# NAIVEddd/MafrixRaytracing

Hardware: AMD Instinct MI355X
Metric: Mrays/s (primary+secondary) at 1080p/64spp; 1/2/4/8-GPU scaling (higher is better)
Workload: dtype f64; 1 GPU; C2 spot (5856 tris) + floor/light stage, 1920x1080, 64 spp per step over 1 GPU(s); scene=scenes/spot.xml, width=1920, height=1080, max_depth=3, frames_in_flight=1, pipeline=wavefront, api=mfx_trace_accumulate of the step's spp (inputs resident in HBM), parallelism=one GPU

## Files before the change

### mafrixraytracing_amd/csrc/mfx_api.cpp

```cpp
#include <dlfcn.h>

#include <mutex>
#include <set>
#include <thread>

#include "mfx_ctx.h"

using namespace mfxh;

namespace {
thread_local std::string g_err;

uint16_t half_dir(float x, bool up) {
    if (std::isinf(x)) return x > 0 ? 0x7c00 : 0xfc00;
    if (x < 0) return (uint16_t)(0x8000 | half_dir(-x, !up));
    if (x == 0) return up ? 0 : 0;
    if (x > 65504.f) return up ? 0x7c00 : 0x7bff;
    int e = 0;
    (void)std::frexp((double)x, &e);
    const int ex = std::max(e - 1, -14);
    const double ulp = std::ldexp(1.0, ex - 10);
    const double m = (double)x / ulp;
    const double k = up ? std::ceil(m) : std::floor(m);
    const double v = k * ulp;
// ... 115 lines not shown
        CK(upload(c->d_nodes_h, nh));
    }
    CK(upload(c->d_slot_ref, c->host.slot_ref));
    CK(upload(c->d_ref_blob, c->host.ref_blob));
    CK(upload(c->d_shade, c->host.shade));
    CK(upload(c->d_albedo, c->host.albedo));
    CK(upload(c->d_light, std::vector<MfxLight>{c->host.light}));
    CK(upload(c->d_cam, std::vector<MfxCamera>{c->host.camera}));
    CK(upload(c->d_refs, std::vector<const void*>{c->d_slot_ref.get(), c->d_ref_blob.get()}));
    const bool inst = !c->host.inst.empty();
    const int ninst = (int)c->host.inst.size();
    if (inst) CK(upload(c->d_inst, c->host.inst));
    const size_t npix = (size_t)c->npix, plane = sizeof(double) * npix;
    CK(c->d_accum_own.alloc(3 * npix));
    c->d_accum = c->d_accum_own;
    CK(c->d_film.alloc(3 * npix));
    CK(c->d_frame.alloc(4 * npix));
    CK(c->d_rgba.alloc(4 * npix));
    CK(c->d_work.alloc(8));
    CK(c->d_counters.alloc(WF_NCTR * WF_SHARDS));
    CK(c->d_counters_total.alloc(WF_NCTR * WF_SHARDS));
    CK(hipMemset(c->d_counters_total, 0, kCounterBytes));
    CK(c->pool.ctl.alloc(WF_CTL_ALLOC));
    size_t mfree = 0, mtotal = 0;
    if (hipMemGetInfo(&mfree, &mtotal) == hipSuccess && mfree > 0)
        c->pool.max = std::max<int64_t>(1 << 20, std::min<int64_t>(c->pool.max, (int64_t)(mfree / 4 / pool_slot_bytes(c))));
    c->pool.fail_once = getenv("MFX_POOL_FAIL_ONCE") && atoi(getenv("MFX_POOL_FAIL_ONCE")) != 0;
    if (const char* pm = getenv("MFX_POOL")) c->pool.max = std::max<int64_t>(2048, std::min<int64_t>(1 << 28, atoll(pm)));
    c->diag_iter = getenv("MFX_DIAG_ITER") != nullptr;
    c->adp.check = getenv("MFX_ADAPTIVE_CHECK") && atoi(getenv("MFX_ADAPTIVE_CHECK")) != 0;
    if (const char* e = getenv("MFX_ITER_EVENTS")) c->iter_events = atoi(e) != 0 || c->diag_iter;
    if (const char* qf = getenv("MFX_QUEUE_FROM")) c->pool.queue_from = MFX_RAY_QUEUE ? std::max(-2, atoi(qf)) : -1;
    if (const char* qc = getenv("MFX_QCHUNK")) c->pool.qchunk = std::max(64, std::min(WF_CHUNK_MAX, atoi(qc) / 64 * 64));
    if (getenv("MFX_RAY_QUEUE") && atoi(getenv("MFX_RAY_QUEUE")) == 0) c->pool.queue_from = -1;
    if (const char* ck = getenv("MFX_MEGA_CHUNK")) c->mega_chunk = std::max(1, atoi(ck));
    if (c->flags & MFX_F_IN_FLIGHT) {
        c->wf_chunk = 512;
        c->wf_shd_half = false;
    }
    if (const char* e = getenv("MFX_SHD_HALF")) c->wf_shd_half = atoi(e) != 0;
    if (const char* ck = getenv("MFX_CHUNK")) c->wf_chunk = std::max(64, std::min(WF_CHUNK_MAX, atoi(ck) / 64 * 64));
    CK(hipMemset(c->d_accum, 0, 3 * plane));
    CK(hipMemset(c->d_film, 0, 3 * plane));
    CK(hipMemset(c->d_counters, 0, kCounterBytes));
    hipDeviceProp_t prop;
    CK(hipGetDeviceProperties(&prop, c->device));
// ... 381 lines not shown
```

### mafrixraytracing_amd/csrc/mfx_ctx.h

```cpp
#pragma once
#include <hip/hip_runtime.h>
#include <rccl/rccl.h>

#include <algorithm>
#include <cmath>
#include <cstdio>
#include <cstdlib>
#include <cstring>
#include <functional>
#include <memory>
#include <string>
#include <utility>
#include <variant>
#include <vector>

#include "../../include/mafrix_rt.h"
#include "mfx_device.h"
#include "mfx_denoise.h"
#include "mfx_scene.h"
#include "mfx_wavefront.h"

namespace mfxh __attribute__((visibility("hidden"))) {

int fail(int code, const std::string& msg);
// ... 116 lines not shown
    decltype(&ncclReduce) reduce = nullptr;
    decltype(&ncclGroupStart) groupStart = nullptr;
    decltype(&ncclGroupEnd) groupEnd = nullptr;
    decltype(&ncclGetErrorString) errorString = nullptr;
};
const Rccl* rccl();

struct WfPool {
    WfParams params{};
    DevBuf<char> mem;
    int32_t slots = 0;
    size_t bytes = 0;
    bool queues = false;
    WfQueue wq[2]{};
    int queue_from = MFX_RAY_QUEUE ? -2 : -1;
    int queue_auto = 1;
    bool auto_read = false;
    bool auto_pending = false;
    int32_t qchunk = 128;
    int64_t max = 1 << 28;
    int64_t cap = 0;
    bool fail_once = false;
    DevBuf<unsigned long long> ctl;
    int queue_start() const { return queue_from == -2 ? queue_auto : queue_from; }
};

struct Ahead {
    int k = 0;
    AheadBuf ab[2];
    int nbuf = 0;
    int cap = 0;
    int cur = -1;
    int64_t last_k = -1;
    uint64_t film_epoch = 1;
    bool film_in_dfilm = true;
    int dfilm_buf = -1;
    int64_t dfilm_n = 0;
    DevBuf<unsigned long long> counters_aux;
    Event aux_ev0, aux_ev1;
    bool ready() const { return nbuf != 0; }
    void release() {
        for (AheadBuf& B : ab) B = AheadBuf{};
        counters_aux.reset(), aux_ev0.reset(), aux_ev1.reset();
        nbuf = cap = 0;
        cur = -1;
    }
// ... 169 lines not shown
```

### mafrixraytracing_amd/csrc/mfx_trace.cpp

```cpp
#include "mfx_ctx.h"

using namespace mfxh;

static int wf_ensure_pool(mfx_ctx* c, int32_t pool, bool queues) {
    WfPool& wp = c->pool;
    if (pool <= wp.slots && (!queues || wp.queues)) return MFX_OK;
    const size_t P = (size_t)pool;
    const int nv = c->host.max_depth + 1;
    const size_t per_slot = pool_slot_bytes(c) - (queues ? 0 : WF_QUEUE_BYTES_PER_SLOT);
    const size_t bytes = P * per_slot + 64 * 256;
    size_t mfree = 0, mtotal = 0, headroom = 0;
    if (hipMemGetInfo(&mfree, &mtotal) == hipSuccess && mfree > 0) {
        const size_t avail = mfree + (wp.mem ? wp.bytes : 0);
        headroom = std::min<size_t>((size_t)2 << 30, avail / 4);
        if (bytes + headroom > avail)
            return fail(MFX_E_NOMEM, "wavefront pool: " + std::to_string(bytes >> 20) + " MiB with " +
                                         std::to_string(avail >> 20) + " MiB free");
    }
    wp.mem.reset();
    wp.slots = 0;
    wp.bytes = 0;
    const hipError_t e = wp.mem.alloc(wp.fail_once ? ((size_t)1 << 50) : bytes);
    wp.fail_once = false;
    if (e != hipSuccess) {
// ... 159 lines not shown
    const int64_t ngen = (total + gen_max - 1) / gen_max;
    const int per_gen = P.max_depth + 1;
    const int iters = (int)ngen * per_gen;
    while (iter_events && (int)c->it_ev.size() < 3 * iters) {
        Event e;
        HIPCHECK(e.create());
        c->it_ev.push_back(std::move(e));
    }
    auto diag = [&](int64_t g, const char* what, int d, float fe, float fs) -> int {
        HIPCHECK(hipStreamSynchronize(c->stream));
        unsigned long long h[WF_NCTR * WF_SHARDS];
        HIPCHECK(hipMemcpy(h, c->d_counters, sizeof(h), hipMemcpyDeviceToHost));
        double r[WF_NCTR] = {0};
        for (int k = 0; k < WF_SHARDS; ++k)
            for (int q = 0; q < WF_NCTR; ++q) r[q] += (double)h[WF_NCTR * k + q];
        for (int q = WF_CTR_ITER + 1; q < WF_CTR_ITER + WF_ITER_CTRS; ++q) r[1] += r[q];
        fprintf(stderr, "gen %lld %s %d: cumulative primary %.0f ext %.0f shadow %.0f; extend %.3f ms shadow %.3f ms;"
                " stamps %.4g %.4g %.4g %.4g outer %.4g node %.4g; cumulative traversal closest %.0f %.0f %.0f"
                " shadow %.0f %.0f %.0f; scan %.4g shade %.4g lat %.4g\n", (long long)g, what, d,
                r[0], r[1], r[2], fe, fs, r[10], r[11], r[12], r[13], r[14], r[15], r[4], r[5], r[6], r[7], r[8], r[9],
                r[16], r[17], r[3]);
        return MFX_OK;
    };
    HIPCHECK(hipEventRecord(fm ? fm->e0 : c->ev0.get(), c->stream));
    int it = 0;
    for (int64_t g = 0; g < ngen; ++g) {
        P.path_base = g * gen_max;
        P.base_smp = P.path_base / per_sample;
        P.base_q = P.path_base % per_sample;
        P.total = std::min<int64_t>(gen_max, total - P.path_base);
        P.pool = (int32_t)((P.total + 4095) / 4096 * 4096);
        HIPCHECK(hipMemsetAsync(P.state, 0, sizeof(int32_t) * (size_t)P.pool, c->stream));
        for (int d = 0; d < per_gen; ++d, ++it) {
            P.start = d == 0 ? 1 : 0;
            P.iter = d;
            wf_queue_views(c, P, d);
            P.chunk = P.qcount ? wp.qchunk : chunk0;
            P.chunk_shd = (c->wf_shd_half && !P.qcount && total <= ((int64_t)1 << 25)) ? std::max(64, P.chunk / 2) : P.chunk;
            if (!iter_events) {
                HIPCHECK(mfx_wf_iteration(P, c->wf_ext_grid, c->wf_shd_grid, stats, c->stream, nullptr));
                continue;
            }
            const Event* ev = c->it_ev.data() + 3 * it;
            hipEvent_t mid = ev[1];
            HIPCHECK(hipEventRecord(ev[0], c->stream));
            HIPCHECK(mfx_wf_iteration(P, c->wf_ext_grid, c->wf_shd_grid, stats, c->stream, &mid));
            HIPCHECK(hipEventRecord(ev[2], c->stream));
            if (c->diag_iter) {
                HIPCHECK(hipStreamSynchronize(c->stream));
                float fe = 0.f, fs = 0.f;
                HIPCHECK(hipEventElapsedTime(&fe, ev[0], ev[1]));
                HIPCHECK(hipEventElapsedTime(&fs, ev[1], ev[2]));
                MFX_TRY(diag(g, "iter", d + 1, fe, fs));
            }
        }
        wf_queue_views(c, P, -1);
        if (split && g == ngen - 1) {
            const int tiles_x = (W + 7) / 8;
            for (int k = 0; k < split->nbands; ++k) {
                const int tx0 = (int)((int64_t)k * tiles_x / split->nbands);
                const int tx1 = (int)((int64_t)(k + 1) * tiles_x / split->nbands);
                P.res_tx0 = tx0;
                P.res_ntx = tx1 - tx0;
                if (P.res_ntx > 0) HIPCHECK(mfx_wf_resolve(P, c->stream));
                MFX_TRY(split->after(k, tx0, tx1 - tx0));
            }
            P.res_tx0 = P.res_ntx = 0;
            split->used = true;
        } else {
            HIPCHECK(mfx_wf_resolve(P, c->stream));
        }
    }
    if (!own_events) {
        HIPCHECK(hipEventRecord(fm->e1, c->stream));
        return MFX_OK;
    }
    HIPCHECK(hipEventRecord(c->ev1, c->stream));
    c->ev_valid = true;
    if (wp.queue_from == -2 && !wp.auto_read) wp.auto_pending = true;
    c->it_recorded = iter_events ? iters : 0;
    c->it_per_gen = per_gen;
    c->generations = (int)ngen;
    return MFX_OK;
}

int mfxh::dev_trace_accumulate(mfx_ctx* c, int32_t spp, int64_t sample_base, ResolveSplit* split) {
    HIPCHECK(hipSetDevice(c->device));
    int64_t ns = spp > c->part_index ? (spp - c->part_index + c->part_count - 1) / c->part_count : 0;
    if (band_rows(c) == 0) ns = 0;
    HIPCHECK(hipMemsetAsync(c->d_work, 0, 64, c->stream));
    HIPCHECK(hipMemsetAsync(c->d_counters, 0, kCounterBytes, c->stream));
    c->mega_last = (c->flags & MFX_F_MEGAKERNEL) != 0 || (ns == 1 && (c->flags & MFX_F_WAVEFRONT) == 0);
    if (ns == 0) {
        HIPCHECK(hipEventRecord(c->ev0, c->stream));
        HIPCHECK(hipEventRecord(c->ev1, c->stream));
        c->ev_valid = true;
        c->it_recorded = 0;
        c->generations = 0;
        return MFX_OK;
    }
    if (!c->mega_last) {
        MFX_TRY(wf_trace(c, ns, sample_base, split ? TraceMode{split} : TraceMode{}));
        HIPCHECK(mfx_launch_counters_add(c->d_counters_total, c->d_counters, WF_NCTR * WF_SHARDS, c->stream));
        return MFX_OK;
    }
    TraceParams P;
    std::memset(&P, 0, sizeof(P));
    fill_trace_params(c, P, sample_base);
    P.work_counter = c->d_work;
    P.counters = c->d_counters;
    P.nsamples = ns;
    P.vscratch = c->d_vscratch;
    P.waves = c->mega_waves;
    if (c->mega_chunk > 0) {
        P.chunk = c->mega_chunk;
    } else {
        const int64_t total = (int64_t)((c->host.width + 7) / 8) * band_rows(c) * 64 * ns;
        int64_t ch = 256;
        while (ch > 64 && total / ch < 16 * (int64_t)c->grid * 4) ch /= 2;
        P.chunk = (int)ch;
    }
    HIPCHECK(hipEventRecord(c->ev0, c->stream));
    HIPCHECK(mfx_launch_trace(P, (c->flags & MFX_F_COUNT_STATS) != 0, c->grid, c->stream));
    HIPCHECK(hipEventRecord(c->ev1, c->stream));
    c->ev_valid = true;
    HIPCHECK(mfx_launch_counters_add(c->d_counters_total, c->d_counters, WF_NCTR * WF_SHARDS, c->stream));
    return MFX_OK;
}

int mfxh::settle_queue_auto(mfx_ctx* c) {
    for (mfx_ctx* d : devs_of(c)) {
// ... 227 lines not shown
```

### mafrixraytracing_amd/csrc/mfx_wavefront.h

```cpp
#ifndef MFX_WAVEFRONT_H
#define MFX_WAVEFRONT_H

#include <hip/hip_runtime.h>
#include <stdint.h>

#include "mfx_layout.h"

#define WF_FREE 0
#define WF_NEED_EXT 1
#define WF_HIT 2
#define WF_MISS 3
#define WF_FRESH 4
#define WF_DONE 8
#define WF_STATE_MASK 15
#define WF_ENTRY_SLOT 0x0fffffff
#define WF_SK_FLAT 0
#define WF_SK_INST 1
#define WF_SK_SLDS 2
#define WF_SHADE_SHIFT 4
#define WF_MAX_VERTS 16
#define WF_LIT_SHIFT 8

#ifndef WF_SHARDS
#define WF_SHARDS 64
#endif
#define WF_CHUNK_MAX 4096
#ifndef WF_LOOKAHEAD
#define WF_LOOKAHEAD 4
#endif
#define WF_NCTR 24
#define WF_CTR_ITER 18
#define WF_ITER_CTRS 6
#ifndef WF_HS
#define WF_HS 32
#endif
#define WF_CTL_EXT 0
#define WF_CTL_SHD (WF_SHARDS * WF_HS)
#define WF_CTL_CLOSED_EXT (2 * WF_SHARDS * WF_HS)
#define WF_CTL_CLOSED_SHD (2 * WF_SHARDS * WF_HS + 16)
#define WF_NCTL (2 * WF_SHARDS * WF_HS + 32)
#define WF_CTL_Q0 (-WF_SHARDS * WF_HS)
#define WF_CTL_Q1 (WF_NCTL)
#define WF_CTL_ALLOC (WF_NCTL + 2 * WF_SHARDS * WF_HS)

typedef uint16_t WfMat;
#define WF_MAT_MAX 65536

struct WfParams {
    const MfxNode* nodes;
    const MfxSlot* slots;
    const int32_t* slot_ref;
    const uint8_t* ref_blob;
    const MfxShade* shade;
    const MfxInstance* inst;
    double tslack;
    MfxLight light;
    const MfxCamera* cam_dev;
#if MFX_NODE_F16
    const MfxNodeH* nodes_h;
#endif
    const MfxLight* light_dev;
    const void* const* refs_dev;
    MfxCamera cam;
    double* accum;
    double* film;
    uint8_t* frames;
// ... 13 lines not shown
    int32_t* state;
    const int32_t* qslot;
    const unsigned long long* qcount;
    int32_t* fstate;
    double *nox, *noy, *noz, *ndx, *ndy, *ndz;
    uint32_t* nrn;
    int32_t *ndepth, *nstate, *nslot;
    unsigned long long* ncount;
    unsigned long long* ctl;
    unsigned long long* counters;
    int64_t total;
    int64_t path_base;
    uint64_t seed;
    int64_t sample_base;
    int32_t part_index, part_count;
    int32_t band_index, band_count, band_rows;
    int32_t pool;
    int32_t width, height, max_depth;
    int32_t stack_size;
    int32_t stack_lds_ext, stack_lds_shd;
    int32_t* spill;
    int32_t chunk;
    int32_t chunk_shd;
    int32_t start;
    int32_t tile_padding;
    int64_t base_smp, base_q;
    int32_t ntop_ext, ntop_shd;
    int32_t nslot_ext, nslot_shd;
    int32_t shadow_waves;
    int32_t ninst_lds;
    int32_t cam_grid;
    int32_t iter;
    int32_t res_tx0, res_ntx;
    const int32_t* tiles;
    int32_t ntiles;
    double* mom;
    const int32_t* tile_n;
    int32_t list_max;
};

struct TileCheckParams {
    const int32_t* tiles;
    int32_t ntiles;
    int32_t n;
    int32_t max_spp;
    int32_t width, height;
// ... 48 lines not shown
```

### mafrixraytracing_amd/csrc/mfx_wavefront.hip

```cpp
#include <hip/hip_runtime.h>
#include <stdint.h>

#include <algorithm>
#include <type_traits>

#include "mfx_device.h"
#include "mfx_trace_common.h"
#include "mfx_wavefront.h"

#ifndef MFX_TRAV_WAVES
#define MFX_TRAV_WAVES 4
#endif

__device__ __forceinline__ int lane_id() { return threadIdx.x & 63; }


#ifndef MFX_SHADOW_ORDER
#define MFX_SHADOW_ORDER 1
#endif

#ifndef MFX_NODE_LANES_MIN
#define MFX_NODE_LANES_MIN 16
#endif
#ifndef MFX_NODE_LANES_MIN_SHD
// ... 29 lines not shown
__device__ __forceinline__ uint64_t lanes_below() { return (1ULL << lane_id()) - 1ULL; }

__device__ __forceinline__ void wave_lds_sync() {
    __builtin_amdgcn_fence(__ATOMIC_RELEASE, "wavefront");
    __builtin_amdgcn_wave_barrier();
    __builtin_amdgcn_fence(__ATOMIC_ACQUIRE, "wavefront");
}

template <int NW>
__device__ __forceinline__ void block_add(unsigned long long* dst, uint32_t v, uint32_t* red) {
    for (int off = 32; off > 0; off >>= 1) v += __shfl_xor(v, off);
    __syncthreads();
    if (lane_id() == 0) red[threadIdx.x >> 6] = v;
    __syncthreads();
    if (threadIdx.x == 0) {
        unsigned long long s = 0;
        for (int w = 0; w < NW; ++w) s += red[w];
        if (s) atomicAdd(dst, s);
    }
}

static_assert(WF_SHARDS == 64, "shard masks are one bit per lane of a wave");

__device__ __forceinline__ uint64_t open_shards(const unsigned long long* ctr, int cap) {
    const unsigned long long v = __hip_atomic_load(ctr + lane_id() * WF_HS, __ATOMIC_RELAXED, __HIP_MEMORY_SCOPE_AGENT);
    return __ballot((int64_t)v < (int64_t)cap);
}

__device__ __forceinline__ int next_open(uint64_t open, int home) {
    const uint64_t r = home ? ((open >> home) | (open << (64 - home))) : open;
    return (home + __builtin_ctzll(r)) & (WF_SHARDS - 1);
}

#ifndef WF_CLOSED_MASK
#define WF_CLOSED_MASK 1
#endif
struct Scanner {
    int win_next, win_end, shard;
    bool exhausted;
    uint64_t closed_seen;
    int b[WF_LOOKAHEAD];
    int nbuf;
    template <bool LOAD = true>
    __device__ __forceinline__ bool window(unsigned long long* heads, int chunk, int shard_size,
                                           const int32_t* __restrict__ state, const unsigned long long* qcount,
                                           unsigned long long* closed) {
        if (win_next < win_end) return true;
        if (exhausted) return false;
        while (true) {
            unsigned long long c = 0;
            if (lane_id() == 0) c = atomicAdd(heads + shard * WF_HS, (unsigned long long)chunk);
            c = __shfl(c, 0);
            const int cap = qcount ? (int)qcount[shard * WF_HS] : shard_size;
            if ((int64_t)c < cap) {
                win_next = shard * shard_size + (int)c;
                win_end = shard * shard_size + min((int)c + chunk, cap);
                if (LOAD) fill(state);
                return true;
            }
#if WF_CLOSED_MASK
            if (lane_id() == 0 && (int64_t)c < (int64_t)cap + chunk) atomicOr(closed, 1ull << shard);
            closed_seen |= 1ull << shard;
            unsigned long long cm = 0;
            if (lane_id() == 0) cm = __hip_atomic_load(closed, __ATOMIC_RELAXED, __HIP_MEMORY_SCOPE_AGENT);
            cm = __shfl(cm, 0);
            const uint64_t open = ~(cm | closed_seen);
#else
            const uint64_t open = open_shards(heads, qcount ? (int)qcount[lane_id() * WF_HS] : shard_size);
#endif
            if (open == 0) {
                exhausted = true;
                return false;
            }
            shard = next_open(open, shard);
        }
    }
    __device__ __forceinline__ void fill(const int32_t* __restrict__ state) {
#pragma unroll
        for (int k = 0; k < WF_LOOKAHEAD; ++k) {
            const int j = win_next + 64 * k + lane_id();
            b[k] = j < win_end ? state[j] : -1;
        }
        nbuf = WF_LOOKAHEAD;
    }
    __device__ __forceinline__ int word() const { return b[0]; }
    __device__ __forceinline__ void advance(const int32_t* __restrict__ state) {
        win_next += 64;
#pragma unroll
        for (int k = 0; k + 1 < WF_LOOKAHEAD; ++k) b[k] = b[k + 1];
        b[WF_LOOKAHEAD - 1] = -1;
        if (--nbuf == 0 && win_next < win_end) fill(state);
    }
};

template <bool SPILL>
__device__ __forceinline__ typename std::conditional<SPILL, SpillStack, LdsStack>::type make_stack(int* lds,
                                                                                                  const WfParams& P,
// ... 237 lines not shown
    double uu = tu, vv = tv;
    if (tu + tv > 1.) { uu = 1. - tu; vv = 1. - tv; }
    const double sq = sqrt(1. - uu);
    const double s1 = 1. - sq, s2 = vv * sq;
    const DV lv0 = lt ? ld3(LT.v0[1]) : ld3(LT.v0[0]);
    const DV le1 = lt ? ld3(LT.e1[1]) : ld3(LT.e1[0]);
    const DV le2 = lt ? ld3(LT.e2[1]) : ld3(LT.e2[0]);
    const DV lp = vadd(vadd(lv0, vmul(le1, s1)), vmul(le2, s2));
    const DV toLight = vsub(lp, hp);
    V.dist = vlen(toLight);
    V.unit = vdiv(toLight, V.dist);
    const double cos_o = vdot(toLight, ld3(LT.normal));
    const double dist2 = toLight.x * toLight.x + toLight.y * toLight.y + toLight.z * toLight.z;
    V.solid = fabs(cos_o) * LT.area / dist2;
    V.cs = vdot(V.unit, nm);
    V.lightable = cos_o < 0.;
    return V;
}

template <bool STATS, bool SPILL, int SK, bool Q, bool START = false, int LIST = WF_LIST_NONE, int NF = MFX_NF_ANY>
__global__ void __launch_bounds__(256, MFX_TRAV_WAVES) k_extend(WfParams P) {
    constexpr bool INST = SK == WF_SK_INST, SLDS = SK == WF_SK_SLDS;
    extern __shared__ int lds_all[];
#if MFX_NODE_F16
    const TopNodes tn{(const float4*)lds_all, P.ntop_ext, P.nodes_h};
#else
    const TopNodes tn{(const float4*)lds_all, P.ntop_ext};
#endif
#if MFX_NODE_F16
    if (NF == MFX_NF_H || (NF == MFX_NF_ANY && P.nodes_h)) load_top_nodes_h((float4*)lds_all, P.nodes_h, P.ntop_ext);
    else
#endif
        load_top_nodes((float4*)lds_all, P.nodes, P.ntop_ext);
    MfxInstance* inst_lds = (MfxInstance*)(lds_all + P.ntop_ext * 32);
    if (INST) load_inst_lds(inst_lds, P.inst, P.ninst_lds);
    int4* slot_lds = (int4*)(inst_lds + (INST ? P.ninst_lds : 0));
    const int nslot = SLDS ? P.nslot_ext : 0;
    if (SLDS) load_slots_lds(slot_lds, P.slots, nslot);
    int* lds = (int*)(slot_lds + 5 * nslot);
    const int lane = lane_id();
    const int wave = threadIdx.x >> 6;
    using Stack = typename std::conditional<SPILL, SpillStack, LdsStack>::type;
    const Stack stack = make_stack<SPILL>(lds + wave * P.stack_lds_ext * 64 + lane, P, P.stack_lds_ext);
    int* pend = lds + 4 * P.stack_lds_ext * 64 + wave * WF_EXT_PEND;
    uint32_t* red = (uint32_t*)(lds + 4 * P.stack_lds_ext * 64 + 4 * WF_EXT_PEND);
    const SceneView S{P.nodes, P.slots, P.slot_ref, P.ref_blob, P.inst, inst_lds, INST ? P.ninst_lds : 0, slot_lds, nslot, nullptr, P.tslack};
// ... 39 lines not shown
    };
    auto finish_ray = [&]() {
        const int s = se & WF_ENTRY_SLOT;
        const bool fresh = START && se < 0;
        const int fl = fresh ? WF_FRESH : 0;
        if (T.B.found) {
            const DV hp = vadd(T.o, vmul(T.d, T.B.t));
            P.ox[s] = hp.x; P.oy[s] = hp.y; P.oz[s] = hp.z;
            const int lm = (P.lit_in_hit && lit_in_entry && !fresh) ? ((se >> 28) & 7) << 29 : 0;
            P.state[s] = ((T.B.info & MFX_INFO_SHADE_MASK) << WF_SHADE_SHIFT) | WF_HIT | fl | lm;
        } else {
            const int lm = fresh || Q ? 0 : (lit_in_entry ? (se >> 28) & 7 : (P.depth[s] >> WF_LIT_SHIFT) & 0xffff);
            P.state[s] = WF_MISS | (lm << WF_SHADE_SHIFT) | fl;
        }
        active = false;
    };

    while (true) {
        bool idle = !active;
        uint64_t m = __ballot(idle);
        while (m != 0) {
            if (pend_lo == pend_hi) {
                int n = 0;
                while (n < 64 && sc.window(P.ctl + WF_CTL_EXT, P.chunk, shard_size, P.state, Q ? P.qcount : nullptr, P.ctl + WF_CTL_CLOSED_EXT)) {
                    if (DG) dg.windows++;
                    const int j = sc.win_next + lane;
                    const int sj = sc.word();
                    bool take = (sj & WF_STATE_MASK) == WF_NEED_EXT;
                    if (START && sj == WF_FREE && j < P.total) {
                        int x, y;
                        int64_t smp;
                        take = !P.tile_padding || path_pixel<LIST>(P, P.path_base + j, x, y, smp);
                    }
                    const uint64_t tm = __ballot(take);
                    if (take)
                        pend[n + __popcll(tm & lanes_below())] =
                            (START && sj == WF_FREE) ? (j | (int)0x80000000)
                                          : (lit_in_entry ? j | (((unsigned)sj >> WF_SHADE_SHIFT) & 7) << 28 : j);
                    n += __popcll(tm);
                    sc.advance(P.state);
                }
                wave_lds_sync();
                pend_lo = 0;
                pend_hi = n;
                c_listed += (uint32_t)n;
                if (n == 0) break;
            }
// ... 26 lines not shown
        atomicAdd(cnt + 11, (unsigned long long)dg.node);
        atomicAdd(cnt + 12, (unsigned long long)dg.leaf);
        atomicAdd(cnt + 13, (unsigned long long)dg.fin);
        atomicAdd(cnt + 14, (unsigned long long)dg.outer);
        atomicAdd(cnt + 3, (unsigned long long)dg.lat);
    }
    if (STATS) {
        block_add<4>(cnt + 4, st.nodes, red);
        block_add<4>(cnt + 5, st.clusters, red);
        block_add<4>(cnt + 6, st.prims, red);
#ifdef MFX_DIAG_OCCLUSION
        block_add<4>(cnt + 13, st.after_nodes, red);
        block_add<4>(cnt + 14, st.after_leaves, red);
#endif
    }
}

#ifndef MFX_CAM_WAVES
#define MFX_CAM_WAVES 5
#endif
template <bool STATS, int LIST = WF_LIST_NONE>
__global__ void __launch_bounds__(256, MFX_CAM_WAVES) k_camera(WfParams P) {
    extern __shared__ int lds_all[];
    const int lane = lane_id();
    const int wave = threadIdx.x >> 6;
    uint64_t* stm = (uint64_t*)lds_all + wave * P.stack_size;
    int* stk = (int*)((uint64_t*)lds_all + 4 * P.stack_size) + wave * P.stack_size;
    uint32_t* red = (uint32_t*)((int*)((uint64_t*)lds_all + 4 * P.stack_size) + 4 * P.stack_size);
    MfxCamera* cam_lds = (MfxCamera*)(red + 16);
    if (threadIdx.x < sizeof(MfxCamera) / 8) ((double*)cam_lds)[threadIdx.x] = ((const double*)P.cam_dev)[threadIdx.x];
    SceneRefs* refs_lds = (SceneRefs*)(cam_lds + 1);
    if (threadIdx.x == 64) *refs_lds = SceneRefs{(const int32_t*)P.refs_dev[0], (const uint8_t*)P.refs_dev[1]};
    __syncthreads();
    const SceneView S{P.nodes, P.slots, nullptr, nullptr, P.inst, nullptr, 0, nullptr, 0, refs_lds};
    const int shard_size = P.pool / WF_SHARDS;
    Scanner sc{};
    sc.shard = blockIdx.x & (WF_SHARDS - 1);
    uint32_t c_primary = 0;
    Stats st{0, 0, 0};
    uint32_t pk_nodes = 0, pk_slots = 0;
#if MFX_DIAG_STAMPS == 3
    uint64_t ph[4] = {0, 0, 0, 0}, t_scan = 0, t_gen = 0, t_out = 0, t_last = stamp();
#define CAM_MARK(acc)                  \
    do {                               \
        const uint64_t _t = stamp();   \
        (acc) += _t - t_last;          \
        t_last = _t;                   \
    } while (0)
#else
#define CAM_MARK(acc) \
    do {              \
    } while (0)
#endif
    while (sc.window<false>(P.ctl + WF_CTL_EXT, P.chunk, shard_size, P.state, nullptr, P.ctl + WF_CTL_CLOSED_EXT)) {
        const int jw = __builtin_amdgcn_readfirstlane(sc.win_next);
        sc.win_next += 64;
        const int j = jw + lane;
        int x = 0, y = 0;
        int64_t smp = 0;
        path_pixel<LIST>(P, P.path_base + jw, x, y, smp);
        x += lane & 7;
        y += lane >> 3;
        const bool act = j < P.total && x < P.width && y < P.height;
        if (!__any(act)) continue;
        CAM_MARK(t_scan);
        DV o = dv(0, 0, 0), d = dv(0, 0, 1);
        if (act) {
            const int64_t pixel = (int64_t)x * P.height + y;
            const int64_t gsample = path_gsample<LIST>(P, smp);
            const uint64_t key = path_key(P.seed, (uint64_t)pixel, (uint64_t)gsample);
            uint32_t rn = 0;
            const double u = ((double)x + rng_next(key, rn)) / (double)P.width;
            const double v = ((double)y + rng_next(key, rn)) / (double)P.height;
            const MfxCamera& CAM = *cam_lds;
            const DV target = vadd(vadd(ld3(CAM.topleft), vmul(ld3(CAM.right), u)), vmul(ld3(CAM.down), v));
            o = ld3(CAM.position);
            d = vnormalize(vsub(target, o));
            c_primary++;
        }
        Best B;
#if MFX_DIAG_STAMPS == 3
        CAM_MARK(t_gen);
        packet_closest<STATS, true>(S, act, o, d, 99999999., B, stk, stm, st, pk_nodes, pk_slots, ph);
        t_last = stamp();
#else
        packet_closest<STATS>(S, act, o, d, 99999999., B, stk, stm, st, pk_nodes, pk_slots);
// ... 52 lines not shown
};
static_assert(sizeof(PixParams) == 72, "PixParams: k_shadow's LDS layout");
struct ShdPtrs {
    double *ox, *oy, *oz, *dx, *dy, *dz, *vei, *vls;
    WfMat* vmat;
    uint32_t* rn;
    int32_t* depth;
    const MfxShade* shade;
    int32_t* fstate;
    const int32_t* qslot;
    double *nox, *noy, *noz, *ndx, *ndy, *ndz;
    uint32_t* nrn;
    int32_t *ndepth, *nstate, *nslot;
    unsigned long long* ncount;
    unsigned long long *ctl, *counters;
    int32_t* state;
    const unsigned long long* qcount;
};

template <bool STATS, bool SPILL, int WAVES, int SK, bool Q, int LIST = WF_LIST_NONE, int NF = MFX_NF_ANY>
__global__ void __launch_bounds__(256, WAVES) k_shadow(WfParams P) {
    constexpr bool INST = SK == WF_SK_INST, SLDS = SK == WF_SK_SLDS;
    extern __shared__ int lds_all[];
#if MFX_NODE_F16
    const TopNodes tn{(const float4*)lds_all, P.ntop_shd, P.nodes_h};
#else
    const TopNodes tn{(const float4*)lds_all, P.ntop_shd};
#endif
    MfxInstance* inst_lds = (MfxInstance*)(lds_all + P.ntop_shd * 32);
    int4* slot_lds = (int4*)(inst_lds + (INST ? P.ninst_lds : 0));
    const int nslot = SLDS ? P.nslot_shd : 0;
    int* lds = (int*)(slot_lds + 5 * nslot);
    uint8_t* pend_base = (uint8_t*)(lds + 4 * P.stack_lds_shd * 64);
    uint32_t* red = (uint32_t*)(pend_base + 4 * PendShd::BYTES);
    MfxLight* light_lds = (MfxLight*)((int*)(red + 16) + 4 * 2 * WF_SHD_LIST);
    if (threadIdx.x < sizeof(MfxLight) / 8)
        ((double*)light_lds)[threadIdx.x] = ((const double*)P.light_dev)[threadIdx.x];
    if (threadIdx.x == 0)
        *(ShdPtrs*)(light_lds + 1) = ShdPtrs{P.ox, P.oy, P.oz, P.dx, P.dy, P.dz, P.vei, P.vls, P.vmat, P.rn, P.depth,
                                            P.shade, P.fstate, P.qslot, P.nox, P.noy, P.noz, P.ndx, P.ndy, P.ndz,
                                            P.nrn, P.ndepth, P.nstate, P.nslot, P.ncount, P.ctl, P.counters, P.state,
                                            P.qcount};
    SceneRefs* refs_lds = (SceneRefs*)((PixParams*)((ShdPtrs*)(light_lds + 1) + 1) + 1);
    if (threadIdx.x == 2)
        *refs_lds = SceneRefs{(const int32_t*)P.refs_dev[0], (const uint8_t*)P.refs_dev[1]};
    if (threadIdx.x == 1) {
// ... 35 lines not shown
    Scanner sc{};
    sc.shard = blockIdx.x & (WF_SHARDS - 1);
    int nshade = 0;
    int pend_lo = 0, pend_hi = 0;
    bool active = false;
    int s = 0;
    Trav T{};
    double scs = 0.0, ssolid = 0.0;
    int vflag = 0;
    uint32_t c_shadow = 0;
    Stats st{0, 0, 0};
#ifdef MFX_DIAG_OCCLUSION
    uint32_t dg_occ = 0, dg_occ_nodes = 0, dg_occ_leaves = 0;
#endif
    constexpr bool DG = MFX_DIAG_STAMPS == 2;
    DiagAcc dg{};
    if (DG) dg.last = stamp();

    while (true) {
        bool idle = !active;
        uint64_t m = __ballot(idle);
        while (m != 0) {
            if (pend_lo == pend_hi) {
                while (nshade < 64 && sc.window(C.ctl + WF_CTL_SHD, P.chunk_shd, shard_size, C.state, Q ? C.qcount : nullptr, C.ctl + WF_CTL_CLOSED_SHD)) {
                    if (DG) dg.windows++;
                    const int j = sc.win_next + lane;
                    const int sj = sc.word();
                    const int sv = sj & WF_STATE_MASK;
                    const bool hit = (sv & ~WF_FRESH) == WF_HIT;
                    if (Q && C.qslot && sv == WF_MISS) {
                        const int dw = C.depth[j];
                        if (dw >> WF_LIT_SHIFT) C.fstate[C.qslot[j]] = WF_DONE | ((dw >> WF_LIT_SHIFT) << WF_SHADE_SHIFT);
                    }
                    const uint64_t hm = __ballot(hit);
                    if (hit) {
                        const int r = nshade + __popcll(hm & lanes_below());
                        const bool lh = P.lit_in_hit && !(Q && C.qslot);
                        shl[r] = (sv & WF_FRESH) ? (j | (int)0x80000000) : (lh ? j | (int)(((unsigned)sj >> 29) << 28) : j);
                        shl[WF_SHD_LIST + r] = (int)(((unsigned)sj >> WF_SHADE_SHIFT) & (lh ? 0x1ffffffu : 0x0fffffffu));
                    }
                    nshade += __popcll(hm);
                    sc.advance(C.state);
                }
                wave_lds_sync();
                DIAG_MARK(dg, scan, DG);
                if (nshade == 0) break;
                const int cnt = nshade < 64 ? nshade : 64;
// ... 501 lines not shown
        switch (scene_kind(inst, P.nslot_ext)) {
            case WF_SK_INST: launch_extend_sk<WF_SK_INST>(P, ext_grid, stats, st, lds_e); break;
            case WF_SK_SLDS: launch_extend_sk<WF_SK_SLDS>(P, ext_grid, stats, st, lds_e); break;
            default: launch_extend_sk<WF_SK_FLAT>(P, ext_grid, stats, st, lds_e);
        }
    }
    if (ev) {
        const hipError_t e = hipEventRecord(ev[0], st);
        if (e != hipSuccess) return e;
    }
    switch (scene_kind(inst, P.nslot_shd)) {
        case WF_SK_INST: launch_shadow_sk<WF_SK_INST>(P, shd_grid, stats, st, lds_s); break;
        case WF_SK_SLDS: launch_shadow_sk<WF_SK_SLDS>(P, shd_grid, stats, st, lds_s); break;
        default: launch_shadow_sk<WF_SK_FLAT>(P, shd_grid, stats, st, lds_s);
    }
    return hipSuccess;
}

hipError_t mfx_wf_iteration(const WfParams& P, int ext_grid, int shd_grid, bool stats, hipStream_t st,
                            hipEvent_t* ev) {
    const int ni = P.inst ? P.ninst_lds : 0;
    const size_t lds_e = wf_lds_bytes(P.stack_lds_ext, false, P.ntop_ext, ni, P.nslot_ext);
    const size_t lds_s = wf_lds_bytes(P.stack_lds_shd, true, P.ntop_shd, ni, P.nslot_shd);
    unsigned long long* z = P.ctl;
    size_t nz = WF_NCTL;
    if (P.ncount) {
        nz += WF_SHARDS * WF_HS;
        if (P.ncount < P.ctl) z = P.ncount;
    }
    hipError_t e = hipMemsetAsync(z, 0, nz * sizeof(unsigned long long), st);
    if (e != hipSuccess) return e;
    e = launch_iteration(P, ext_grid, shd_grid, stats, st, ev, lds_e, lds_s);
    if (e != hipSuccess) return e;
    return hipGetLastError();
}

hipError_t mfx_wf_resolve(const WfParams& P, hipStream_t st) {
    if (P.mom || P.ntiles > 0) {
        if (!P.mom || P.film || P.res_ntx > 0) return hipErrorInvalidValue;
        const int64_t n = P.ntiles > 0 ? (int64_t)P.ntiles * 64 : (int64_t)((P.width + 7) >> 3) * P.band_rows * 64;
        hipLaunchKernelGGL(k_resolve<WF_RES_MOMENTS>, dim3((unsigned)((n + 255) / 256)), dim3(256), 0, st, P);
        return hipGetLastError();
    }
    const int64_t per_sample = (int64_t)(P.res_ntx > 0 ? P.res_ntx : (P.width + 7) >> 3) * P.band_rows * 64;
    if (P.film) hipLaunchKernelGGL(k_resolve<WF_RES_FRAMES>, dim3((unsigned)((per_sample + 255) / 256)), dim3(256), 0, st, P);
    else hipLaunchKernelGGL(k_resolve<WF_RES_ACCUM>, dim3((unsigned)((per_sample + 255) / 256)), dim3(256), 0, st, P);
    return hipGetLastError();
}

__device__ __forceinline__ double wave_sum(double v) {
    for (int off = 32; off > 0; off >>= 1) v += __shfl_xor(v, off);
    return v;
}

__device__ __forceinline__ bool tile_converged(const TileCheckParams& C, int T, int ni, int& m) {
// ... 106 lines not shown
```

Baseline: 12020 Mrays/s.

## Taper work-stealing windows at shard tails and zero control words in kernels

```diff
diff --git a/mafrixraytracing_amd/csrc/mfx_api.cpp b/mafrixraytracing_amd/csrc/mfx_api.cpp
--- a/mafrixraytracing_amd/csrc/mfx_api.cpp
+++ b/mafrixraytracing_amd/csrc/mfx_api.cpp
@@ -161,6 +161,8 @@
     CK(c->d_counters_total.alloc(WF_NCTR * WF_SHARDS));
     CK(hipMemset(c->d_counters_total, 0, kCounterBytes));
     CK(c->pool.ctl.alloc(WF_CTL_ALLOC));
+    CK(hipMemset(c->pool.ctl, 0, sizeof(unsigned long long) * WF_CTL_ALLOC));
+    if (const char* e = getenv("MFX_TAPER")) c->pool.tail_windows = std::max(0, std::min(64, atoi(e)));
     size_t mfree = 0, mtotal = 0;
     if (hipMemGetInfo(&mfree, &mtotal) == hipSuccess && mfree > 0)
         c->pool.max = std::max<int64_t>(1 << 20, std::min<int64_t>(c->pool.max, (int64_t)(mfree / 4 / pool_slot_bytes(c))));
diff --git a/mafrixraytracing_amd/csrc/mfx_ctx.h b/mafrixraytracing_amd/csrc/mfx_ctx.h
--- a/mafrixraytracing_amd/csrc/mfx_ctx.h
+++ b/mafrixraytracing_amd/csrc/mfx_ctx.h
@@ -162,6 +162,8 @@
     int64_t cap = 0;
     bool fail_once = false;
     DevBuf<unsigned long long> ctl;
+    bool ctl_dirty = false;
+    int32_t tail_windows = WF_TAIL_WINDOWS;
     int queue_start() const { return queue_from == -2 ? queue_auto : queue_from; }
 };
 
diff --git a/mafrixraytracing_amd/csrc/mfx_trace.cpp b/mafrixraytracing_amd/csrc/mfx_trace.cpp
--- a/mafrixraytracing_amd/csrc/mfx_trace.cpp
+++ b/mafrixraytracing_amd/csrc/mfx_trace.cpp
@@ -205,6 +205,9 @@
                 r[16], r[17], r[3]);
         return MFX_OK;
     };
+    if (wp.ctl_dirty) HIPCHECK(hipMemsetAsync(wp.ctl, 0, sizeof(unsigned long long) * WF_CTL_ALLOC, c->stream));
+    wp.ctl_dirty = true;
+    const bool cam_starts = P.cam_grid > 0 && !P.inst;
     HIPCHECK(hipEventRecord(fm ? fm->e0 : c->ev0.get(), c->stream));
     int it = 0;
     for (int64_t g = 0; g < ngen; ++g) {
@@ -213,11 +216,13 @@
         P.base_q = P.path_base % per_sample;
         P.total = std::min<int64_t>(gen_max, total - P.path_base);
         P.pool = (int32_t)((P.total + 4095) / 4096 * 4096);
-        HIPCHECK(hipMemsetAsync(P.state, 0, sizeof(int32_t) * (size_t)P.pool, c->stream));
+        if (!cam_starts) HIPCHECK(hipMemsetAsync(P.state, 0, sizeof(int32_t) * (size_t)P.pool, c->stream));
         for (int d = 0; d < per_gen; ++d, ++it) {
             P.start = d == 0 ? 1 : 0;
             P.iter = d;
             wf_queue_views(c, P, d);
+            P.tail_ext = wf_tail_slots(d == 0 && cam_starts ? P.cam_grid : c->wf_ext_grid, wp.tail_windows);
+            P.tail_shd = wf_tail_slots(c->wf_shd_grid, wp.tail_windows);
             P.chunk = P.qcount ? wp.qchunk : chunk0;
             P.chunk_shd = (c->wf_shd_half && !P.qcount && total <= ((int64_t)1 << 25)) ? std::max(64, P.chunk / 2) : P.chunk;
             if (!iter_events) {
@@ -254,6 +259,7 @@
             HIPCHECK(mfx_wf_resolve(P, c->stream));
         }
     }
+    wp.ctl_dirty = false;
     if (!own_events) {
         HIPCHECK(hipEventRecord(fm->e1, c->stream));
         return MFX_OK;
@@ -271,7 +277,6 @@
     HIPCHECK(hipSetDevice(c->device));
     int64_t ns = spp > c->part_index ? (spp - c->part_index + c->part_count - 1) / c->part_count : 0;
     if (band_rows(c) == 0) ns = 0;
-    HIPCHECK(hipMemsetAsync(c->d_work, 0, 64, c->stream));
     HIPCHECK(hipMemsetAsync(c->d_counters, 0, kCounterBytes, c->stream));
     c->mega_last = (c->flags & MFX_F_MEGAKERNEL) != 0 || (ns == 1 && (c->flags & MFX_F_WAVEFRONT) == 0);
     if (ns == 0) {
@@ -290,6 +295,7 @@
     TraceParams P;
     std::memset(&P, 0, sizeof(P));
     fill_trace_params(c, P, sample_base);
+    HIPCHECK(hipMemsetAsync(c->d_work, 0, 64, c->stream));
     P.work_counter = c->d_work;
     P.counters = c->d_counters;
     P.nsamples = ns;
diff --git a/mafrixraytracing_amd/csrc/mfx_wavefront.h b/mafrixraytracing_amd/csrc/mfx_wavefront.h
--- a/mafrixraytracing_amd/csrc/mfx_wavefront.h
+++ b/mafrixraytracing_amd/csrc/mfx_wavefront.h
@@ -42,6 +42,43 @@
 #define WF_CTL_Q0 (-WF_SHARDS * WF_HS)
 #define WF_CTL_Q1 (WF_NCTL)
 #define WF_CTL_ALLOC (WF_NCTL + 2 * WF_SHARDS * WF_HS)
+
+struct WfTaper {
+    int nb;
+    int body;
+    int nt;
+};
+__host__ __device__ inline WfTaper wf_taper(int cap, int chunk, int tail) {
+    WfTaper T;
+    const unsigned rest = cap > tail ? (unsigned)(cap - tail) : 0u;
+    T.nb = (int)(rest / (unsigned)chunk);
+    T.body = T.nb * chunk;
+    T.nt = cap > 0 ? T.nb + (cap - T.body + 63) / 64 : 0;
+    return T;
+}
+__host__ __device__ inline bool wf_ticket_range(unsigned long long t, int cap, int chunk, int tail, int* begin, int* end,
+                                                bool* closes) {
+    const WfTaper T = wf_taper(cap, chunk, tail);
+    *closes = t == (unsigned long long)T.nt;
+    if (t >= (unsigned long long)T.nt) return false;
+    const int k = (int)t;
+    const int b = k < T.nb ? k * chunk : T.body + (k - T.nb) * 64;
+    const int e = b + (k < T.nb ? chunk : 64);
+    *begin = b;
+    *end = e < cap ? e : cap;
+    return true;
+}
+__host__ __device__ inline int wf_next_open(uint64_t open, int home) {
+    const uint64_t r = home ? ((open >> home) | (open << (64 - home))) : open;
+    return (home + __builtin_ctzll(r)) & (WF_SHARDS - 1);
+}
+#ifndef WF_TAIL_WINDOWS
+#define WF_TAIL_WINDOWS 2
+#endif
+inline int wf_tail_slots(int grid, int windows) {
+    const int waves = grid * 4 / WF_SHARDS;
+    return 64 * windows * (waves > 1 ? waves : 1);
+}
 
 typedef uint16_t WfMat;
 #define WF_MAT_MAX 65536
@@ -101,6 +138,7 @@
     int32_t* spill;
     int32_t chunk;
     int32_t chunk_shd;
+    int32_t tail_ext, tail_shd;
     int32_t start;
     int32_t tile_padding;
     int64_t base_smp, base_q;
diff --git a/mafrixraytracing_amd/csrc/mfx_wavefront.hip b/mafrixraytracing_amd/csrc/mfx_wavefront.hip
--- a/mafrixraytracing_amd/csrc/mfx_wavefront.hip
+++ b/mafrixraytracing_amd/csrc/mfx_wavefront.hip
@@ -75,19 +75,14 @@
 
 static_assert(WF_SHARDS == 64, "shard masks are one bit per lane of a wave");
 
-__device__ __forceinline__ uint64_t open_shards(const unsigned long long* ctr, int cap) {
-    const unsigned long long v = __hip_atomic_load(ctr + lane_id() * WF_HS, __ATOMIC_RELAXED, __HIP_MEMORY_SCOPE_AGENT);
-    return __ballot((int64_t)v < (int64_t)cap);
-}
-
-__device__ __forceinline__ int next_open(uint64_t open, int home) {
-    const uint64_t r = home ? ((open >> home) | (open << (64 - home))) : open;
-    return (home + __builtin_ctzll(r)) & (WF_SHARDS - 1);
-}
-
-#ifndef WF_CLOSED_MASK
-#define WF_CLOSED_MASK 1
-#endif
+__device__ __forceinline__ void zero_ctl_words(unsigned long long* heads, unsigned long long* closed,
+                                               unsigned long long* counts) {
+    if (blockIdx.x != 0 || threadIdx.x >= WF_SHARDS) return;
+    __hip_atomic_store(heads + threadIdx.x * WF_HS, 0ull, __ATOMIC_RELAXED, __HIP_MEMORY_SCOPE_AGENT);
+    if (counts) __hip_atomic_store(counts + threadIdx.x * WF_HS, 0ull, __ATOMIC_RELAXED, __HIP_MEMORY_SCOPE_AGENT);
+    if (threadIdx.x == 0) __hip_atomic_store(closed, 0ull, __ATOMIC_RELAXED, __HIP_MEMORY_SCOPE_AGENT);
+}
+
 struct Scanner {
     int win_next, win_end, shard;
     bool exhausted;
@@ -95,37 +90,35 @@
     int b[WF_LOOKAHEAD];
     int nbuf;
     template <bool LOAD = true>
-    __device__ __forceinline__ bool window(unsigned long long* heads, int chunk, int shard_size,
+    __device__ __forceinline__ bool window(unsigned long long* heads, int chunk, int tail, int shard_size,
                                            const int32_t* __restrict__ state, const unsigned long long* qcount,
                                            unsigned long long* closed) {
         if (win_next < win_end) return true;
         if (exhausted) return false;
         while (true) {
-            unsigned long long c = 0;
-            if (lane_id() == 0) c = atomicAdd(heads + shard * WF_HS, (unsigned long long)chunk);
-            c = __shfl(c, 0);
+            unsigned long long t = 0;
+            if (lane_id() == 0) t = atomicAdd(heads + shard * WF_HS, 1ull);
+            t = __shfl(t, 0);
             const int cap = qcount ? (int)qcount[shard * WF_HS] : shard_size;
-            if ((int64_t)c < cap) {
-                win_next = shard * shard_size + (int)c;
-                win_end = shard * shard_size + min((int)c + chunk, cap);
+            int rb, re;
+            bool closes;
+            if (wf_ticket_range(t, cap, chunk, tail, &rb, &re, &closes)) {
+                win_next = shard * shard_size + rb;
+                win_end = shard * shard_size + re;
                 if (LOAD) fill(state);
                 return true;
             }
-#if WF_CLOSED_MASK
-            if (lane_id() == 0 && (int64_t)c < (int64_t)cap + chunk) atomicOr(closed, 1ull << shard);
+            if (lane_id() == 0 && closes) atomicOr(closed, 1ull << shard);
             closed_seen |= 1ull << shard;
             unsigned long long cm = 0;
             if (lane_id() == 0) cm = __hip_atomic_load(closed, __ATOMIC_RELAXED, __HIP_MEMORY_SCOPE_AGENT);
             cm = __shfl(cm, 0);
             const uint64_t open = ~(cm | closed_seen);
-#else
-            const uint64_t open = open_shards(heads, qcount ? (int)qcount[lane_id() * WF_HS] : shard_size);
-#endif
             if (open == 0) {
                 exhausted = true;
                 return false;
             }
-            shard = next_open(open, shard);
+            shard = wf_next_open(open, shard);
         }
     }
     __device__ __forceinline__ void fill(const int32_t* __restrict__ state) {
@@ -409,6 +402,7 @@
 __global__ void __launch_bounds__(256, MFX_TRAV_WAVES) k_extend(WfParams P) {
     constexpr bool INST = SK == WF_SK_INST, SLDS = SK == WF_SK_SLDS;
     extern __shared__ int lds_all[];
+    zero_ctl_words(P.ctl + WF_CTL_SHD, P.ctl + WF_CTL_CLOSED_SHD, P.ncount);
 #if MFX_NODE_F16
     const TopNodes tn{(const float4*)lds_all, P.ntop_ext, P.nodes_h};
 #else
@@ -494,7 +488,7 @@
         while (m != 0) {
             if (pend_lo == pend_hi) {
                 int n = 0;
-                while (n < 64 && sc.window(P.ctl + WF_CTL_EXT, P.chunk, shard_size, P.state, Q ? P.qcount : nullptr, P.ctl + WF_CTL_CLOSED_EXT)) {
+                while (n < 64 && sc.window(P.ctl + WF_CTL_EXT, P.chunk, P.tail_ext, shard_size, P.state, Q ? P.qcount : nullptr, P.ctl + WF_CTL_CLOSED_EXT)) {
                     if (DG) dg.windows++;
                     const int j = sc.win_next + lane;
                     const int sj = sc.word();
@@ -567,6 +561,7 @@
 template <bool STATS, int LIST = WF_LIST_NONE>
 __global__ void __launch_bounds__(256, MFX_CAM_WAVES) k_camera(WfParams P) {
     extern __shared__ int lds_all[];
+    zero_ctl_words(P.ctl + WF_CTL_SHD, P.ctl + WF_CTL_CLOSED_SHD, P.ncount);
     const int lane = lane_id();
     const int wave = threadIdx.x >> 6;
     uint64_t* stm = (uint64_t*)lds_all + wave * P.stack_size;
@@ -597,7 +592,7 @@
     do {              \
     } while (0)
 #endif
-    while (sc.window<false>(P.ctl + WF_CTL_EXT, P.chunk, shard_size, P.state, nullptr, P.ctl + WF_CTL_CLOSED_EXT)) {
+    while (sc.window<false>(P.ctl + WF_CTL_EXT, P.chunk, P.tail_ext, shard_size, P.state, nullptr, P.ctl + WF_CTL_CLOSED_EXT)) {
         const int jw = __builtin_amdgcn_readfirstlane(sc.win_next);
         sc.win_next += 64;
         const int j = jw + lane;
@@ -607,6 +602,7 @@
         x += lane & 7;
         y += lane >> 3;
         const bool act = j < P.total && x < P.width && y < P.height;
+        if (!act) P.state[j] = WF_FREE;
         if (!__any(act)) continue;
         CAM_MARK(t_scan);
         DV o = dv(0, 0, 0), d = dv(0, 0, 1);
@@ -705,6 +701,7 @@
 __global__ void __launch_bounds__(256, WAVES) k_shadow(WfParams P) {
     constexpr bool INST = SK == WF_SK_INST, SLDS = SK == WF_SK_SLDS;
     extern __shared__ int lds_all[];
+    zero_ctl_words(P.ctl + WF_CTL_EXT, P.ctl + WF_CTL_CLOSED_EXT, nullptr);
 #if MFX_NODE_F16
     const TopNodes tn{(const float4*)lds_all, P.ntop_shd, P.nodes_h};
 #else
@@ -786,7 +783,7 @@
         uint64_t m = __ballot(idle);
         while (m != 0) {
             if (pend_lo == pend_hi) {
-                while (nshade < 64 && sc.window(C.ctl + WF_CTL_SHD, P.chunk_shd, shard_size, C.state, Q ? C.qcount : nullptr, C.ctl + WF_CTL_CLOSED_SHD)) {
+                while (nshade < 64 && sc.window(C.ctl + WF_CTL_SHD, P.chunk_shd, P.tail_shd, shard_size, C.state, Q ? C.qcount : nullptr, C.ctl + WF_CTL_CLOSED_SHD)) {
                     if (DG) dg.windows++;
                     const int j = sc.win_next + lane;
                     const int sj = sc.word();
@@ -1334,15 +1331,7 @@
     const int ni = P.inst ? P.ninst_lds : 0;
     const size_t lds_e = wf_lds_bytes(P.stack_lds_ext, false, P.ntop_ext, ni, P.nslot_ext);
     const size_t lds_s = wf_lds_bytes(P.stack_lds_shd, true, P.ntop_shd, ni, P.nslot_shd);
-    unsigned long long* z = P.ctl;
-    size_t nz = WF_NCTL;
-    if (P.ncount) {
-        nz += WF_SHARDS * WF_HS;
-        if (P.ncount < P.ctl) z = P.ncount;
-    }
-    hipError_t e = hipMemsetAsync(z, 0, nz * sizeof(unsigned long long), st);
-    if (e != hipSuccess) return e;
-    e = launch_iteration(P, ext_grid, shd_grid, stats, st, ev, lds_e, lds_s);
+    const hipError_t e = launch_iteration(P, ext_grid, shd_grid, stats, st, ev, lds_e, lds_s);
     if (e != hipSuccess) return e;
     return hipGetLastError();
 }
diff --git a/mafrixraytracing_amd/csrc/taper_check.cpp b/mafrixraytracing_amd/csrc/taper_check.cpp
--- /dev/null
+++ b/mafrixraytracing_amd/csrc/taper_check.cpp
@@ -0,0 +1,165 @@
+#include <cstdio>
+#include <cstdlib>
+#include <random>
+#include <vector>
+
+#include "mfx_wavefront.h"
+
+static int failures = 0;
+#define CHECK(cond, ...)                      \
+    do {                                      \
+        if (!(cond)) {                        \
+            if (++failures <= 20) {           \
+                fprintf(stderr, "FAIL: ");    \
+                fprintf(stderr, __VA_ARGS__); \
+                fprintf(stderr, "\n");        \
+            }                                 \
+        }                                     \
+    } while (0)
+
+static void check_closed_form(int cap, int chunk, int tail) {
+    std::vector<unsigned char> seen((size_t)(cap > 0 ? cap : 0), 0);
+    const WfTaper T = wf_taper(cap, chunk, tail);
+    CHECK(T.nt >= 0 && T.nt <= (cap > 0 ? cap : 0) / 64 + 1, "ticket count %d for cap %d", T.nt, cap);
+    for (long long t = 0; t <= (long long)T.nt + 2; ++t) {
+        int b = -1, e = -1;
+        bool closes = false;
+        const bool ok = wf_ticket_range((unsigned long long)t, cap, chunk, tail, &b, &e, &closes);
+        CHECK(ok == (t < T.nt), "cap %d chunk %d tail %d ticket %lld: has slots %d", cap, chunk, tail, t, (int)ok);
+        CHECK(closes == (t == T.nt), "cap %d chunk %d tail %d ticket %lld: closes %d", cap, chunk, tail, t, (int)closes);
+        if (!ok) continue;
+        CHECK(b % 64 == 0 && b < e && e <= cap && e - b <= chunk, "cap %d chunk %d tail %d ticket %lld: [%d, %d)", cap,
+              chunk, tail, t, b, e);
+        for (int j = b; j < e && j < cap; ++j) {
+            CHECK(j >= 0 && !seen[(size_t)j], "cap %d chunk %d tail %d: slot %d twice", cap, chunk, tail, j);
+            if (j >= 0) seen[(size_t)j] = 1;
+        }
+    }
+    for (int j = 0; j < cap; ++j) CHECK(seen[(size_t)j], "cap %d chunk %d tail %d: slot %d never", cap, chunk, tail, j);
+}
+
+struct Wave {
+    int shard;
+    bool exhausted = false;
+    uint64_t closed_seen = 0;
+    int phase = 0;
+    bool closes = false;
+    int failed = 0;
+    long long fetched = 0;
+};
+
+static void simulate(int blocks, int shard_size, int chunk, int tail, const int* caps, std::mt19937_64& rng) {
+    unsigned long long heads[WF_SHARDS] = {0};
+    unsigned long long closed = 0;
+    int closed_sets[WF_SHARDS] = {0};
+    std::vector<unsigned char> seen((size_t)WF_SHARDS * shard_size, 0);
+    std::vector<Wave> waves((size_t)blocks * 4);
+    for (size_t w = 0; w < waves.size(); ++w) waves[w].shard = (int)((w / 4) & (WF_SHARDS - 1));
+    std::vector<int> live(waves.size());
+    for (size_t w = 0; w < waves.size(); ++w) live[w] = (int)w;
+    long long total_cap = 0, total_tickets = 0;
+    for (int g = 0; g < WF_SHARDS; ++g) {
+        const int cap = caps ? caps[g] : shard_size;
+        total_cap += cap;
+        total_tickets += wf_taper(cap, chunk, tail).nt;
+    }
+    const long long step_bound = 3 * (total_tickets + 64LL * (long long)waves.size()) + 16;
+    long long steps = 0;
+    while (!live.empty() && steps <= step_bound) {
+        ++steps;
+        const size_t pick = (size_t)(rng() % live.size());
+        Wave& W = waves[(size_t)live[pick]];
+        if (W.phase == 0) {
+            const unsigned long long t = heads[W.shard]++;
+            const int cap = caps ? caps[W.shard] : shard_size;
+            int b, e;
+            if (wf_ticket_range(t, cap, chunk, tail, &b, &e, &W.closes)) {
+                ++W.fetched;
+                CHECK(b % 64 == 0 && e - b <= chunk && e <= cap, "range [%d, %d) of shard %d", b, e, W.shard);
+                for (int j = b; j < e; ++j) {
+                    unsigned char& s = seen[(size_t)W.shard * shard_size + j];
+                    CHECK(!s, "slot %d of shard %d handed out twice", j, W.shard);
+                    s = 1;
+                }
+                continue;
+            }
+            ++W.failed;
+            W.phase = 1;
+        } else if (W.phase == 1) {
+            if (W.closes) {
+                closed |= 1ull << W.shard;
+                ++closed_sets[W.shard];
+            }
+            W.closed_seen |= 1ull << W.shard;
+            W.phase = 2;
+        } else {
+            const uint64_t open = ~(closed | W.closed_seen);
+            W.phase = 0;
+            if (open == 0) {
+                W.exhausted = true;
+                live[pick] = live.back();
+                live.pop_back();
+            } else {
+                W.shard = wf_next_open(open, W.shard);
+            }
+        }
+    }
+    CHECK(live.empty(), "%zu waves not exhausted after %lld steps (blocks %d shard %d chunk %d tail %d)", live.size(), steps,
+          blocks, shard_size, chunk, tail);
+    long long handed = 0;
+    for (int g = 0; g < WF_SHARDS; ++g) {
+        const int cap = caps ? caps[g] : shard_size;
+        for (int j = 0; j < shard_size; ++j) {
+            const bool s = seen[(size_t)g * shard_size + j] != 0;
+            handed += s;
+            CHECK(s == (j < cap), "shard %d slot %d (cap %d): handed out %d (chunk %d tail %d)", g, j, cap, (int)s, chunk, tail);
+        }
+        CHECK(closed_sets[g] <= 1, "shard %d: closed bit set %d times", g, closed_sets[g]);
+    }
+    CHECK(handed == total_cap, "handed out %lld of %lld slots", handed, total_cap);
+    for (const Wave& W : waves) CHECK(W.failed <= WF_SHARDS, "a wave failed %d fetches", W.failed);
+}
+
+int main() {
+    std::mt19937_64 rng(20240611);
+    const int chunks[] = {64, 128, 256, 1024, 4096};
+    const int tails[] = {0, 64, 128, 1024, 8192, 1 << 22};
+    long long cases = 0;
+    for (int chunk : chunks)
+        for (int tail : tails) {
+            const int caps[] = {0, 1, 63, 64, 65, chunk - 1, chunk, chunk + 1, 2 * chunk + 65, tail, tail + 1, tail + chunk - 1,
+                                tail + chunk, tail + chunk + 1, 100000};
+            for (int cap : caps)
+                if (cap <= (1 << 22)) {
+                    check_closed_form(cap, chunk, tail);
+                    ++cases;
+                }
+        }
+    const int shard_sizes[] = {64, 128, 320, 4096, 20032};
+    const int grids[] = {1, 3, 16, 64, 200};
+    for (int chunk : chunks)
+        for (int tail : tails)
+            for (int shard_size : shard_sizes)
+                for (int blocks : grids) {
+                    if (tail > 8192 && shard_size < 4096) continue;
+                    simulate(blocks, shard_size, chunk, tail, nullptr, rng);
+                    int caps[WF_SHARDS];
+                    const int edge[] = {0, 1, 63, 64, 65, chunk - 1, chunk, chunk + 1, shard_size - 1, shard_size};
+                    for (int g = 0; g < WF_SHARDS; ++g) {
+                        int cap = g < 10 ? edge[g] : (int)(rng() % (unsigned)(shard_size + 1));
+                        caps[g] = cap < 0 ? 0 : cap > shard_size ? shard_size : cap;
+                    }
+                    simulate(blocks, shard_size, chunk, tail, caps, rng);
+                    for (int g = 0; g < WF_SHARDS; ++g) caps[g] = (g % 7 == 3) ? 1 : 0;
+                    simulate(blocks, shard_size, chunk, tail, caps, rng);
+                    for (int g = 0; g < WF_SHARDS; ++g) caps[g] = 0;
+                    simulate(blocks, shard_size, chunk, tail, caps, rng);
+                    cases += 4;
+                }
+    if (failures) {
+        fprintf(stderr, "taper_check: %d failures in %lld cases\n", failures, cases);
+        return 1;
+    }
+    printf("taper_check ok: %lld cases\n", cases);
+    return 0;
+}
```

After: 12050 Mrays/s, median of 6. No clear change (+0.2%).
